# krukah/robopoker

Measured on AMD Instinct MI355X. Metric: mccfr_infoset_updates_per_sec, higher is better.
Workload: dtype f32; 1 GPU; leduc-holdem external-sampling MCCFR, tables resident in HBM (BASELINE configs[1]); regret=floored, weight=linear, sampling=external, batch_per_gpu=8388608, global_batch=8388608, infosets=120, actions=2, update=composed, parallelism=tree-sharded x1

## Files before the change

### robopoker_amd/csrc/mccfr.hip

```cpp
#include "mccfr_kernels.hpp"
#include "mccfr_traverse.hpp"
#include "mccfr_update.hpp"
#include "traverse_static.hpp"
#include "mccfr_nash.hpp"
#include "host_util.hpp"

#include <algorithm>
#include <chrono>
#include <cstdlib>
#include <functional>
#include <string>
#include <type_traits>
#include <vector>

using namespace rp;

namespace {
const char* const CLOCK_NAMES[] = {"traverse", "compact", "update"};
enum { CK_TRAVERSE, CK_COMPACT, CK_UPDATE, CK_COUNT };
}

struct rp_mccfr {
    int device = 0;
    hipStream_t stream = nullptr;
// ... 86 lines not shown
    if (h->d_dec) HIP_TRY(hipFree(h->d_dec));
    h->d_scratch = h->d_dec = nullptr;
    const size_t stride = ((size_t)batch + 255) & ~(size_t)255;
    const uint32_t A = h->tbl.max_actions;
    DevScratch& sc = h->sc;
    sc.stride = stride;
    const size_t node_words = (size_t)sc.maxn * stride, stack_words = (size_t)sc.maxs * stride;
    const size_t total_words = 8 * node_words + 4 * stack_words + (size_t)A * stride;
    HIP_TRY(hipMalloc(&h->d_scratch, total_words * 4));
    uint32_t* base = reinterpret_cast<uint32_t*>(h->d_scratch);
    sc.n_meta = base; base += node_words;
    sc.n_info = base; base += node_words;
    sc.n_frel = reinterpret_cast<float*>(base); base += node_words;
    sc.n_fsmp = reinterpret_cast<float*>(base); base += node_words;
    sc.n_pay = reinterpret_cast<float*>(base); base += node_words;
    sc.n_rel = reinterpret_cast<float*>(base); base += node_words;
    sc.n_smp = reinterpret_cast<float*>(base); base += node_words;
    sc.n_acc = reinterpret_cast<float*>(base); base += node_words;
    sc.s_state = base; base += stack_words;
    sc.s_meta = base; base += stack_words;
    sc.s_frel = reinterpret_cast<float*>(base); base += stack_words;
    sc.s_fsmp = reinterpret_cast<float*>(base); base += stack_words;
    sc.t_v = reinterpret_cast<float*>(base);

    DevDecisions& dc = h->dc;
    dc.stride = stride;
    dc.maxdec = h->maxdec;
    const size_t slot_words = (size_t)dc.maxdec * stride;
    const bool small = chunk_maps_lds_bytes(h) <= 64 * 1024 && h->tbl.n_infos <= CM_PASSES * CH_THREADS && !getenv("RP_MCCFR_SLOTMAP");
    const size_t dec_bytes = (3 * slot_words + 2 * slot_words * A) * 4 + (small ? 0 : (size_t)h->tbl.n_infos * stride) + stride;
    HIP_TRY(hipMalloc(&h->d_dec, dec_bytes));
    uint32_t* d = reinterpret_cast<uint32_t*>(h->d_dec);
    dc.info = d; d += slot_words;
    dc.mask = d; d += slot_words;
    dc.payoff = reinterpret_cast<float*>(d); d += slot_words;
    dc.regret = reinterpret_cast<float*>(d); d += slot_words * A;
    dc.policy = reinterpret_cast<float*>(d); d += slot_words * A;
    dc.ndec = reinterpret_cast<uint8_t*>(d);
    dc.slotmap = small ? nullptr : dc.ndec + stride;
    if (h->d_sorted) HIP_TRY(hipFree(h->d_sorted));
    h->d_sorted = nullptr;
    DevSorted& so = h->so;
    so.n_chunks = (uint32_t)((stride + CH_TREES - 1) / CH_TREES);
    const size_t cap = slot_words;
    const size_t nic = (size_t)h->tbl.n_infos * so.n_chunks;
    const size_t sorted_words = cap * 2 * A + 2 * cap + 2 * nic + h->tbl.n_infos;
    HIP_TRY(hipMalloc(&h->d_sorted, sorted_words * 4));
    uint32_t* sw = reinterpret_cast<uint32_t*>(h->d_sorted);
    so.rw = reinterpret_cast<float*>(sw); sw += cap * 2 * A;
    so.mask = sw; sw += cap;
    so.payoff = reinterpret_cast<float*>(sw); sw += cap;
    so.counts = sw; sw += nic;
    so.offs = sw; sw += nic;
    so.total = sw;
    if (h->d_bmaps) HIP_TRY(hipFree(h->d_bmaps));
    h->d_bmaps = nullptr;
    const size_t nblk_max = (stride + RP_COMPOSE_CHUNK - 1) / RP_COMPOSE_CHUNK;
    const size_t ngrp_max = (nblk_max + RP_FOLD_GROUP - 1) / RP_FOLD_GROUP;
    const size_t bytes = bmap_index((uint32_t)(nblk_max + ngrp_max), 0, 0, h->g.rank_max, 2 * A) * sizeof(Map) + (size_t)h->tbl.n_infos * sizeof(uint32_t);
    HIP_TRY(hipMalloc(&h->d_bmaps, bytes));
    HIP_TRY(hipMemset(h->d_bmaps, 0, bytes));
    HIP_TRY(hipDeviceSynchronize());
    h->capacity = batch;
    return RP_OK;
}

StepParams make_params(const rp_mccfr* h) {
    StepParams p{};
    p.seed = h->seed;
    p.epoch = h->epoch;
    p.tree_base = (uint64_t)h->rank * h->batch;
    p.batch = h->batch;
    p.walker = (uint32_t)(h->epoch % h->tbl.n_players);
    p.R = h->R; p.W = h->W; p.S = h->S;
    p.temperature = h->hp.temperature; p.smoothing = h->hp.smoothing; p.curiosity = h->hp.curiosity;
    p.prune_threshold = h->hp.prune_threshold; p.prune_explore = h->hp.prune_explore;
    p.prune_warmup = h->hp.prune_warmup;
    p.regret_min = h->hp.regret_min;
    if (h->R == RP_REGRET_DISCOUNTED) {
        p.pow15 = rp_pow15((float)h->epoch);
        p.pow05 = rp_pow05((float)h->epoch);
    }
    p.counters = h->d_counters;
    if (h->rng == RP_RNG_REFERENCE) {
        p.ref_info = reinterpret_cast<const rp_sip_mid*>(h->d_ref_mid);
        p.ref_chance = p.ref_info + h->tbl.n_infos;
    }
    return p;
}

template <class F>
void with_bool(bool a, F&& f) {
    if (a) f(std::true_type{});
    else f(std::false_type{});
}
template <class F>
void with_bools(bool a, bool b, F&& f) {
    with_bool(a, [&](auto ta) { with_bool(b, [&](auto tb) { f(ta, tb); }); });
}

template <class F>
void with_skeleton(int static_skel, F&& f) {
    if (static_skel == 1) f(KuhnSkel{});
    else if (static_skel == 2) f(LeducSkel{});
}
template <class F>
void with_static_traversal(int static_skel, uint32_t walker, bool pruned, bool ref, F&& f) {
    with_skeleton(static_skel, [&](auto gt) {
        with_bool(walker == 0, [&](auto w0) {
            with_bools(pruned, ref, [&](auto pr, auto rf) { f(gt, std::integral_constant<int, decltype(w0)::value ? 0 : 1>{}, pr, rf); });
        });
    });
}

template <class G>
bool skel_matches(const rp_game_table* game, const std::vector<uint32_t>& children) {
    constexpr Skeleton S = SkelOf<G>::S;
    if (game->n_players != 2 || game->max_actions != 2) return false;
    std::vector<std::vector<int>> kids(S.n);
    for (int s = 1; s < S.n; ++s) kids[S.parent[s]].push_back(s);
    std::vector<int> node_of_info(game->n_infos, -1);
    std::function<bool(uint32_t, int)> match = [&](uint32_t sid, int s) -> bool {
        const rp_state& st = game->states[sid];
        if (S.kind[s] == SK_TERMINAL) return st.n_children == 0;
        if (S.kind[s] == SK_CHANCE) {
            if (st.turn != RP_TURN_CHANCE || st.n_children == 0 || kids[s].size() != 1) return false;
            for (uint32_t k = 0; k < st.n_children; ++k)
                if (!match(children[st.offset + k], kids[s][0])) return false;
            return true;
        }
        if (st.turn != (uint8_t)(S.kind[s] - SK_P0) || st.n_children != 2 || kids[s].size() != 2 || st.info >= game->n_infos) return false;
        if (node_of_info[st.info] >= 0 && node_of_info[st.info] != s) return false;
        node_of_info[st.info] = s;
        for (int c : kids[s])
            if (S.edge[c] > 1 || !match(children[st.offset + (uint32_t)S.edge[c]], c)) return false;
        return kids[s][0] != kids[s][1] && S.edge[kids[s][0]] != S.edge[kids[s][1]];
    };
    return match(game->train_root, 0);
}

template <class G>
bool build_rows(const rp_game_table* game, const std::vector<uint32_t>& children, const std::function<uint4(uint32_t)>& rec_of,
                std::vector<uint32_t>& rows, uint32_t* base, uint32_t* fan) {
    constexpr Skeleton S = SkelOf<G>::S;
    constexpr RowLayout R = SkelOf<G>::R;
    std::vector<std::vector<int>> kids(S.n);
    for (int s = 1; s < S.n; ++s) kids[S.parent[s]].push_back(s);
    for (int s = 0; s < S.n; ++s) fan[s] = base[s] = 0;
    bool uniform = true;
    std::function<void(uint32_t, int)> fans = [&](uint32_t sid, int s) {
        const rp_state& st = game->states[sid];
        if (S.kind[s] == SK_CHANCE) {
            if (fan[s] == 0) fan[s] = st.n_children;
            else if (fan[s] != st.n_children) uniform = false;
            for (uint32_t k = 0; k < st.n_children; ++k) fans(children[st.offset + k], kids[s][0]);
        } else if (S.kind[s] != SK_TERMINAL) {
            for (int c : kids[s]) fans(children[st.offset + (uint32_t)S.edge[c]], c);
        }
    };
    fans(game->train_root, 0);
    if (!uniform) return false;
    uint64_t total = 0;
    for (int c = 0; c < S.n; ++c) {
        if (S.kind[c] != SK_CHANCE) continue;
        uint64_t count = 1;
        for (int a = 0; a <= c; ++a)
            if (S.kind[a] == SK_CHANCE && c <= S.end[a]) count *= fan[a];
        base[c] = (uint32_t)(total / 4);
        total += (count * (uint64_t)R.stride[c] + 31) & ~(uint64_t)31;
        if (total > (1ull << 28)) return false;
    }
    rows.assign(total, 0u);
    std::function<void(uint32_t, int, uint64_t)> fill = [&](uint32_t sid, int s, uint64_t idx) {
        const rp_state& st = game->states[sid];
        if (const int c = R.group[s]; c >= 0) {
            uint32_t* row = &rows[(size_t)base[c] * 4 + idx * (uint64_t)R.stride[c]];
            const uint4 r = rec_of(sid);
            if (S.kind[s] == SK_CHANCE) {
                row[R.word[s]] = r.w;
                row[R.word2[s]] = r.y;
            } else if (S.kind[s] == SK_TERMINAL) {
                row[R.word[s]] = r.y;
                row[R.word2[s]] = r.z;
            } else {
                row[R.word[s]] = r.y;
            }
        }
        if (S.kind[s] == SK_CHANCE) {
            for (uint32_t k = 0; k < st.n_children; ++k) fill(children[st.offset + k], kids[s][0], idx * fan[s] + k);
        } else if (S.kind[s] != SK_TERMINAL) {
            for (int c : kids[s]) fill(children[st.offset + (uint32_t)S.edge[c]], c, idx);
        }
    };
    fill(game->train_root, 0, 0);
    return true;
}

size_t traverse_lds_bytes(const rp_mccfr* h) {
    const size_t shared = std::max<size_t>(2 * (size_t)h->maxint, 4 * (size_t)h->sc.maxs);
    return ((size_t)2 * h->sc.maxn + shared + (h->tbl.max_actions <= 4 ? 0 : h->tbl.max_actions)) * 64 * 4;
}
bool traverse_fits_lds(const rp_mccfr* h) {
    return h->sc.maxn <= 62 && h->maxint <= 32 && h->tbl.max_depth <= 10 && h->tbl.n_infos <= 8191 && h->tbl.max_actions <= 16 &&
           traverse_lds_bytes(h) <= 64 * 1024;
}

void launch_prepare_ref(rp_mccfr* h, const StepParams& p) {
    if (h->rng == RP_RNG_REFERENCE && h->ref_mid_epoch != p.epoch) {
        const uint32_t n = h->tbl.n_infos + h->n_chance_infos;
        rp_sip_mid* mid = reinterpret_cast<rp_sip_mid*>(h->d_ref_mid);
        hipLaunchKernelGGL(k_prepare_ref, dim3((n + 63) / 64), dim3(64), 0, h->stream, reinterpret_cast<const rp_hash_stream*>(h->d_info_streams),
                           h->tbl.n_infos, reinterpret_cast<const rp_hash_stream*>(h->d_chance_streams), h->n_chance_infos, p.epoch, mid,
                           mid + h->tbl.n_infos);
        h->ref_mid_epoch = p.epoch;
    }
}
void launch_prepare(rp_mccfr* h, const StepParams& p) {
    launch_prepare_ref(h, p);
    if (h->itab_version == h->tables_version) return;
    hipLaunchKernelGGL(k_prepare_infos, dim3((h->tbl.n_infos + 63) / 64), dim3(64), 0, h->stream, h->g, h->t, p, h->itab);
    h->itab_version = h->tables_version;
}

int launch_traverse(rp_mccfr* h, const StepParams& p) {
    if (h->dc.slotmap) HIP_TRY(hipMemsetAsync(h->dc.slotmap, 0, (size_t)h->tbl.n_infos * h->dc.stride, h->stream));
    h->clk.begin(h->stream, CK_TRAVERSE);
    if (h->static_skel) {
        launch_prepare(h, p);
        const dim3 grid((h->batch + 255) / 256), block(256);
        with_static_traversal(h->static_skel, p.walker, p.S != RP_SAMPLING_EXTERNAL, p.ref_info != nullptr, [&](auto gt, auto wk, auto pr, auto rf) {
            hipLaunchKernelGGL((k_traverse_static<decltype(gt), decltype(wk)::value, decltype(pr)::value, decltype(rf)::value>), grid, block, 0,
                               h->stream, h->g, h->itab, h->dc, p);
        });
    } else if (h->use_lds_traverse) {
        launch_prepare(h, p);
        const size_t lds = traverse_lds_bytes(h);
        const dim3 grid((h->batch + 63) / 64), block(64);
        with_bool(h->tbl.max_actions <= 4, [&](auto tv) {
            hipLaunchKernelGGL((k_traverse_lds<decltype(tv)::value>), grid, block, lds, h->stream, h->g, h->itab, h->dc, p, h->sc.maxn, h->sc.maxs,
                               h->maxint);
        });
    } else {
        launch_prepare_ref(h, p);
        const uint32_t threads = 256, blocks = (h->batch + threads - 1) / threads;
        hipLaunchKernelGGL(k_traverse, dim3(blocks), dim3(threads), 0, h->stream, h->g, h->t, h->sc, h->dc, p);
    }
    h->clk.end(h->stream, CK_TRAVERSE);
    HIP_TRY(hipGetLastError());
    return RP_OK;
}

int launch_sort(rp_mccfr* h, const StepParams& p) {
    const uint32_t nchunks = (h->batch + CH_TREES - 1) / CH_TREES;
    h->so.n_chunks = nchunks;
    h->clk.begin(h->stream, CK_COMPACT);
    if (!h->dc.slotmap) {
        const size_t NI = h->tbl.n_infos;
        hipLaunchKernelGGL(k_count_small, dim3(nchunks), dim3(CH_THREADS), NI * SM_WORDS * 4, h->stream, h->g, h->dc, h->so, p);
        hipLaunchKernelGGL(k_scan, dim3(h->tbl.n_infos), dim3(CH_THREADS), 0, h->stream, h->g, h->so, p);
        hipLaunchKernelGGL(k_compact_small, dim3(nchunks), dim3(CH_THREADS), NI * SM_WORDS * 4 + 2 * NI * 4 + NI * SM_WORDS * 2,
                           h->stream, h->g, h->dc, h->so, p);
    } else {
        hipLaunchKernelGGL(k_count, dim3(nchunks, h->tbl.n_infos), dim3(SLOT_THREADS), 0, h->stream, h->g, h->dc, h->so, p);
        hipLaunchKernelGGL(k_scan, dim3(h->tbl.n_infos), dim3(CH_THREADS), 0, h->stream, h->g, h->so, p);
        hipLaunchKernelGGL(k_compact, dim3(nchunks, h->tbl.n_infos), dim3(SLOT_THREADS), 0, h->stream, h->g, h->dc, h->so, p);
    }
    h->clk.end(h->stream, CK_COMPACT);
    HIP_TRY(hipGetLastError());
    return RP_OK;
}

int launch_chain(rp_mccfr* h, const StepParams& p) {
    const size_t lds = chain_lds_bytes();
    const bool sgn = h->R == RP_REGRET_DISCOUNTED || h->R == RP_REGRET_ASYMMETRIC;
    const bool prn = h->S != RP_SAMPLING_EXTERNAL;
    const dim3 grid(h->tbl.n_infos), block(128);
    h->clk.begin(h->stream, CK_UPDATE);
    with_bools(sgn, prn, [&](auto sg, auto pr) {
        hipLaunchKernelGGL((k_chain<decltype(sg)::value, decltype(pr)::value>), grid, block, lds, h->stream, h->g, h->t, h->so, p);
    });
    h->clk.end(h->stream, CK_UPDATE);
    HIP_TRY(hipGetLastError());
    return RP_OK;
}

uint32_t chunks_of(size_t trees) { return (uint32_t)((trees + RP_COMPOSE_CHUNK - 1) / RP_COMPOSE_CHUNK); }
size_t chunk_maps_lds_bytes(const rp_mccfr* h) {
    const size_t NI = h->tbl.n_infos;
    return NI * SM_WORDS * 4 + 2 * NI * 4 + (size_t)CH_TREES * h->maxdec * 4 + NI * SM_WORDS * 2 +
           2 * (size_t)CH_TREES * h->maxdec * 2;
}

size_t traverse_maps_lds_bytes(const rp_mccfr* h) {
    const size_t NI = h->tbl.n_infos;
    const size_t masks = h->S != RP_SAMPLING_EXTERNAL ? (size_t)h->maxdec * 256 * 4 : 0;
    return (NI * 8 + 2 * NI) * 4 + NI * 8 * 2 + (NI + (NI & 1)) * 2 + 2 * NI * 4 + (size_t)3 * (h->maxdec * 256 + h->cell_pad) * 4 + masks;
}
static_assert(CH_THREADS <= 256u, "k_traverse_maps_static packs (infoset, rank of the infoset) into the 16 bits of an `order` entry");
bool traverse_maps_fused(const rp_mccfr* h) {
    return h->static_skel && !h->dc.slotmap && h->tbl.n_infos <= CH_THREADS && h->g.rank_max <= 64u &&
           traverse_maps_lds_bytes(h) <= 64 * 1024 && h->fuse_maps;
}

constexpr uint32_t FOLD_SPLIT_GROUPS = 128;
bool fold_split(const rp_mccfr* h, uint32_t batch) {
    const uint32_t ngrp = (chunks_of(batch) + RP_FOLD_GROUP - 1) / RP_FOLD_GROUP;
    return ngrp >= h->fold_split_groups;
}

int launch_summarize(rp_mccfr* h, const StepParams& p, void* blob_dev, bool fused = false, bool apply = false) {
    unsigned char* blob = reinterpret_cast<unsigned char*>(blob_dev);
    Cell* cells = reinterpret_cast<Cell*>(blob);
    InfoSum* sums = reinterpret_cast<InfoSum*>(blob + (size_t)h->tbl.n_infos * h->tbl.max_actions * sizeof(Cell));
    const uint32_t A = h->tbl.max_actions;
    const uint32_t nblk_max = chunks_of(h->dc.stride), nblk = chunks_of(h->batch);
    Map* bmaps = reinterpret_cast<Map*>(h->d_bmaps);
    const bool pruned = h->S != RP_SAMPLING_EXTERNAL;
    if (fused) {
        h->clk.begin(h->stream, CK_TRAVERSE);
        launch_prepare(h, p);
        const size_t lds = traverse_maps_lds_bytes(h);
        with_static_traversal(h->static_skel, p.walker, pruned, p.ref_info != nullptr, [&](auto gt, auto wk, auto pr, auto rf) {
            hipLaunchKernelGGL((k_traverse_maps_static<decltype(gt), decltype(wk)::value, decltype(pr)::value, decltype(rf)::value>), dim3(nblk),
                               dim3(256), lds, h->stream, h->g, h->itab, p, bmaps, h->maxdec, h->cell_pad);
        });
        h->clk.end(h->stream, CK_TRAVERSE);
    }
    h->clk.begin(h->stream, CK_UPDATE);
    if (fused) {
    } else if (!h->dc.slotmap) {
        const size_t lds = chunk_maps_lds_bytes(h);
        with_bools(pruned, h->tbl.n_infos <= CH_THREADS, [&](auto pr, auto one) {
            hipLaunchKernelGGL((k_chunk_maps<decltype(pr)::value, decltype(one)::value ? 1u : CM_PASSES>), dim3(nblk), dim3(CH_THREADS), lds,
                               h->stream, h->g, h->dc, p, bmaps);
        });
    } else {
        with_bool(pruned, [&](auto pr) {
            hipLaunchKernelGGL((k_block_maps<decltype(pr)::value>), dim3(nblk, h->tbl.n_infos), dim3(128), 0, h->stream, h->g, h->so, p, bmaps);
        });
    }
    {
        const uint32_t W2 = 2 * A, nr = h->g.rank_count[p.walker];
        const uint32_t ngrp_max = (nblk_max + RP_FOLD_GROUP - 1) / RP_FOLD_GROUP, ngrp = (nblk + RP_FOLD_GROUP - 1) / RP_FOLD_GROUP;
        FoldScratch fs;
        fs.gmaps = bmaps + bmap_index(nblk_max, 0, 0, h->g.rank_max, W2);
        fs.done = reinterpret_cast<uint32_t*>(bmaps + bmap_index(nblk_max + ngrp_max, 0, 0, h->g.rank_max, W2));
        const dim3 grid(std::max(ngrp, 1u), cb2_tiles(nr, W2)), fold_grid(std::max(nr, 1u));
        const bool split = fold_split(h, h->batch);
        if (split) hipLaunchKernelGGL((k_combine2<false, false>), grid, dim3(CB2_THREADS), 0, h->stream, h->g, h->t, h->itab, p, bmaps, nr, fs, cells, sums);
        if (apply) {
            if (split) hipLaunchKernelGGL((k_fold_groups<true>), fold_grid, dim3(CB2_THREADS), 0, h->stream, h->g, h->t, h->itab, p, fs.gmaps, nr, cells, sums);
            else hipLaunchKernelGGL((k_combine2<true>), grid, dim3(CB2_THREADS), 0, h->stream, h->g, h->t, h->itab, p, bmaps, nr, fs, cells, sums);
            h->tables_version += 1;
            if (h->itab_version + 1 == h->tables_version) h->itab_version = h->tables_version;
        } else {
            if (split) hipLaunchKernelGGL((k_fold_groups<false>), fold_grid, dim3(CB2_THREADS), 0, h->stream, h->g, h->t, h->itab, p, fs.gmaps, nr, cells, sums);
            else hipLaunchKernelGGL((k_combine2<false>), grid, dim3(CB2_THREADS), 0, h->stream, h->g, h->t, h->itab, p, bmaps, nr, fs, cells, sums);
        }
    }
    h->clk.end(h->stream, CK_UPDATE);
    HIP_TRY(hipGetLastError());
    return RP_OK;
}

int launch_batch_summary(rp_mccfr* h, const StepParams& p, void* blob_dev, bool apply = false) {
    if (traverse_maps_fused(h)) return launch_summarize(h, p, blob_dev, true, apply);
    int rc = launch_traverse(h, p);
    if (rc) return rc;
    if (h->dc.slotmap && (rc = launch_sort(h, p))) return rc;
    return launch_summarize(h, p, blob_dev, false, apply);
}

int enqueue_step(rp_mccfr* h) {
    const StepParams p = make_params(h);
    int rc;
    if (h->mode == RP_UPDATE_ORDERED) {
        if ((rc = launch_traverse(h, p))) return rc;
        if ((rc = launch_sort(h, p))) return rc;
        if ((rc = launch_chain(h, p))) return rc;
        h->tables_version += 1;
    } else {
        if ((rc = launch_batch_summary(h, p, h->d_summary, true))) return rc;
    }
    h->epoch += 1;
    return RP_OK;
}

int read_counters(rp_mccfr* h, unsigned long long c[3]) {
    std::vector<unsigned long long> all((size_t)METRIC_STRIPES * METRIC_STRIDE);
    HIP_TRY(hipMemcpyAsync(all.data(), h->d_counters, all.size() * 8, hipMemcpyDeviceToHost, h->stream));
    HIP_TRY(hipStreamSynchronize(h->stream));
    c[0] = c[1] = c[2] = 0;
    for (uint32_t s = 0; s < METRIC_STRIPES; ++s) {
        c[0] += all[(size_t)s * METRIC_STRIDE];
        c[1] += all[(size_t)s * METRIC_STRIDE + 1];
        c[2] |= all[(size_t)s * METRIC_STRIDE + 2];
    }
    return RP_OK;
}

int check_device_errors(rp_mccfr* h) {
    unsigned long long c[3];
    int rc = read_counters(h, c);
    if (rc) return rc;
    if (c[2]) return rp::fail(RP_ERR_CAPACITY, "mccfr kernel capacity exceeded (flags %llu): nodes/stack/decisions", c[2]);
    return RP_OK;
}

int composed_supported(const rp_mccfr* h) {
    if (h->R == RP_REGRET_DISCOUNTED || h->R == RP_REGRET_ASYMMETRIC)
        return rp::fail(RP_ERR_UNSUPPORTED,
                        "composed update needs a sign-independent discount (Summed/Linear/Floored regret)");
    return RP_OK;
}

int fetch_tables(rp_mccfr* h, std::vector<float>& regret, std::vector<float>& weight, std::vector<float>& payoff,
                 std::vector<uint32_t>& visits) {
    const size_t cells = (size_t)h->tbl.n_infos * h->tbl.max_actions;
    regret.resize(cells); weight.resize(cells); payoff.resize(cells); visits.resize(cells);
    HIP_TRY(hipMemcpyAsync(regret.data(), h->t.regret, cells * 4, hipMemcpyDeviceToHost, h->stream));
    HIP_TRY(hipMemcpyAsync(weight.data(), h->t.weight, cells * 4, hipMemcpyDeviceToHost, h->stream));
    HIP_TRY(hipMemcpyAsync(payoff.data(), h->t.payoff, cells * 4, hipMemcpyDeviceToHost, h->stream));
    HIP_TRY(hipMemcpyAsync(visits.data(), h->t.visits, cells * 4, hipMemcpyDeviceToHost, h->stream));
    HIP_TRY(hipStreamSynchronize(h->stream));
    return RP_OK;
}

}

extern "C" {

int rp_mccfr_create(const rp_game_table* game, rp_regret_kind r, rp_weight_kind w, rp_sampling_kind s,
                    uint32_t batch_size, const rp_hyper* hp, uint64_t seed, int device, rp_mccfr** out) {
    if (!game || !out) return rp::fail(RP_ERR_INVALID, "rp_mccfr_create: NULL argument");
    int rc = rp_game_table_check(game);
    if (rc) return rc;
    if ((int)r < 0 || (int)r > 4 || (int)w < 0 || (int)w > 3 || (int)s < 0 || (int)s > 2)
        return rp::fail(RP_ERR_INVALID, "rp_mccfr_create: unknown schedule / sampling kind");
    if (batch_size == 0) return rp::fail(RP_ERR_INVALID, "rp_mccfr_create: batch_size must be > 0");
    if (rp_device_count() <= 0)
        return rp::fail(RP_ERR_NO_DEVICE, "rp_mccfr_create: no HIP device visible; the MI355X path has no CPU fallback");
    if (game->max_tree_nodes == 0 || game->max_tree_nodes >= 255)
        return rp::fail(RP_ERR_CAPACITY, "rp_mccfr_create: sampled trees of up to %u nodes exceed the per-lane limit (254)",
                        game->max_tree_nodes);
    rp_mccfr* h = new rp_mccfr();
    h->device = device;
    h->tbl = *game;
    h->states.assign(game->states, game->states + game->n_states);
    h->children.assign(game->children, game->children + game->n_children);
    h->payoffs.assign(game->payoffs, game->payoffs + (size_t)game->n_terminals * game->n_players);
    h->info_actions.assign(game->info_actions, game->info_actions + game->n_infos);
    h->info_player.assign(game->info_player, game->info_player + game->n_infos);
    const size_t cells = (size_t)game->n_infos * game->max_actions;
    h->default_regret.assign(cells, 0.0f);
    if (game->default_regret) h->default_regret.assign(game->default_regret, game->default_regret + cells);
    h->tbl.states = h->states.data();
    h->tbl.children = h->children.data();
    h->tbl.payoffs = h->payoffs.data();
    h->tbl.info_actions = h->info_actions.data();
    h->tbl.info_player = h->info_player.data();
    h->tbl.default_regret = h->default_regret.data();
    h->R = r; h->W = w; h->S = s;
    if (hp) h->hp = *hp; else rp_hyper_default(&h->hp);
    h->seed = seed;
    h->batch = batch_size;

#define CREATE_TRY(expr)                                                                             \
    do {                                                                                             \
        hipError_t _e = (expr);                                                                      \
        if (_e != hipSuccess) {                                                                      \
            int _rc = rp::fail(RP_ERR_HIP, "%s failed: %s", #expr, hipGetErrorString(_e));           \
            rp_mccfr_destroy(h);                                                                     \
            return _rc;                                                                              \
        }                                                                                            \
    } while (0)

    CREATE_TRY(hipSetDevice(device));
    CREATE_TRY(hipStreamCreateWithFlags(&h->stream, hipStreamNonBlocking));
    h->own_stream = true;
    std::vector<uint4> packed(game->n_states);
    for (uint32_t i = 0; i < game->n_states; ++i) {
        const rp_state& st = game->states[i];
        packed[i] = make_uint4((uint32_t)st.turn | ((uint32_t)st.n_children << 8), st.turn == RP_TURN_CHANCE ? (uint32_t)st.chance_info : st.info, st.offset, 0u);
    }
    CREATE_TRY(hipMalloc(&h->d_states, packed.size() * sizeof(uint4)));
    CREATE_TRY(hipMemcpy(h->d_states, packed.data(), packed.size() * sizeof(uint4), hipMemcpyHostToDevice));
    CREATE_TRY(hipMalloc(&h->d_children, h->children.size() * 4));
    CREATE_TRY(hipMemcpy(h->d_children, h->children.data(), h->children.size() * 4, hipMemcpyHostToDevice));
    const std::function<uint4(uint32_t)> rec_of = [&](uint32_t sid) {
        uint4 r = packed[sid];
        r.w = sid;
        if (game->states[sid].n_children == 0 && game->n_players == 2) {
            r.y = rp_f2u(h->payoffs[(size_t)game->states[sid].offset * 2 + 0]);
            r.z = rp_f2u(h->payoffs[(size_t)game->states[sid].offset * 2 + 1]);
        }
        return r;
    };
    std::vector<uint4> kids(h->children.size());
    for (size_t c = 0; c < h->children.size(); ++c) kids[c] = rec_of(h->children[c]);
    CREATE_TRY(hipMalloc(&h->d_kids, std::max<size_t>(kids.size(), 1) * sizeof(uint4)));
    CREATE_TRY(hipMemcpy(h->d_kids, kids.data(), kids.size() * sizeof(uint4), hipMemcpyHostToDevice));
    CREATE_TRY(hipMalloc(&h->d_payoffs, h->payoffs.size() * 4));
    CREATE_TRY(hipMemcpy(h->d_payoffs, h->payoffs.data(), h->payoffs.size() * 4, hipMemcpyHostToDevice));
    CREATE_TRY(hipMalloc(&h->d_info_actions, game->n_infos));
    CREATE_TRY(hipMemcpy(h->d_info_actions, h->info_actions.data(), game->n_infos, hipMemcpyHostToDevice));
    CREATE_TRY(hipMalloc(&h->d_info_player, game->n_infos));
    CREATE_TRY(hipMemcpy(h->d_info_player, h->info_player.data(), game->n_infos, hipMemcpyHostToDevice));
    h->g.states = reinterpret_cast<const uint4*>(h->d_states);
    h->g.children = reinterpret_cast<const uint32_t*>(h->d_children);
    h->g.kids = reinterpret_cast<const uint4*>(h->d_kids);
    h->g.root_rec = packed[game->train_root];
    h->g.root_rec.w = game->train_root;
    h->g.payoffs = reinterpret_cast<const float*>(h->d_payoffs);
    h->g.info_actions = reinterpret_cast<const uint8_t*>(h->d_info_actions);
    h->g.info_player = reinterpret_cast<const uint8_t*>(h->d_info_player);
    {
        std::vector<uint32_t> rank(game->n_infos), count(8, 0u);
        const auto owned = [&](uint32_t i) { return h->info_player[i] < game->n_players; };
        for (uint32_t i = 0; i < game->n_infos; ++i) rank[i] = owned(i) ? count[h->info_player[i]]++ : 0u;
        uint32_t rank_max = 1;
        for (uint32_t w = 0; w < 8; ++w) {
            h->g.rank_count[w] = count[w];
            rank_max = std::max(rank_max, count[w]);
        }
        h->g.rank_max = rank_max;
        std::vector<uint32_t> tab((size_t)game->n_infos + (size_t)game->n_players * rank_max, 0u);
        for (uint32_t i = 0; i < game->n_infos; ++i) {
            tab[i] = rank[i];
            if (owned(i)) tab[(size_t)game->n_infos + (size_t)h->info_player[i] * rank_max + rank[i]] = i;
        }
        CREATE_TRY(hipMalloc(&h->d_info_rank, tab.size() * 4));
        CREATE_TRY(hipMemcpy(h->d_info_rank, tab.data(), tab.size() * 4, hipMemcpyHostToDevice));
        h->g.info_rank = reinterpret_cast<const uint32_t*>(h->d_info_rank);
        h->g.rank_info = h->g.info_rank + game->n_infos;
    }
    h->g.n_players = game->n_players;
    h->g.n_infos = game->n_infos;
    h->g.A = game->max_actions;
    h->g.root = game->train_root;
    CREATE_TRY(hipMalloc(&h->t.regret, cells * 4));
    CREATE_TRY(hipMalloc(&h->t.weight, cells * 4));
    CREATE_TRY(hipMalloc(&h->t.payoff, cells * 4));
    CREATE_TRY(hipMalloc(&h->t.visits, cells * 4));
    CREATE_TRY(hipMemcpy(h->t.regret, h->default_regret.data(), cells * 4, hipMemcpyHostToDevice));
    CREATE_TRY(hipMemset(h->t.weight, 0, cells * 4));
    CREATE_TRY(hipMemset(h->t.payoff, 0, cells * 4));
    CREATE_TRY(hipMemset(h->t.visits, 0, cells * 4));
    CREATE_TRY(hipMalloc(&h->d_counters, (size_t)METRIC_STRIPES * METRIC_STRIDE * sizeof(unsigned long long)));
    CREATE_TRY(hipMemset(h->d_counters, 0, (size_t)METRIC_STRIPES * METRIC_STRIDE * sizeof(unsigned long long)));
    CREATE_TRY(hipMalloc(&h->d_summary, summary_bytes_of(h)));
    CREATE_TRY(hipMalloc(&h->d_itab, (5 * cells + 2 * (size_t)game->n_infos + 4 + 8 * (size_t)game->n_infos + 8) * 4));
    {
        float* f = reinterpret_cast<float*>(h->d_itab);
        h->itab.sigma = f;
        h->itab.q = f + cells;
        h->itab.cum = f + 2 * cells;
        h->itab.total = f + 3 * cells;
        h->itab.keep = reinterpret_cast<uint32_t*>(f + 3 * cells + game->n_infos);
        const size_t used = 3 * cells + 2 * (size_t)game->n_infos;
        h->itab.sq = reinterpret_cast<float2*>(f + ((used + 3) & ~(size_t)3));
        const size_t used2 = ((used + 3) & ~(size_t)3) + 2 * cells;
        h->itab.row2 = game->max_actions == 2 ? f + ((used2 + 7) & ~(size_t)7) : nullptr;
    }
    uint32_t maxstack = 1;
    sampled_tree_bounds(h, &h->maxdec, &maxstack, &h->maxint);
    h->sc.maxn = game->max_tree_nodes;
    h->sc.maxs = maxstack;
    if (h->maxdec > 254) {
        rp_mccfr_destroy(h);
        return rp::fail(RP_ERR_CAPACITY, "rp_mccfr_create: more than 254 walker infosets per tree");
    }
    if (chain_lds_bytes() > 64 * 1024) {
        rp_mccfr_destroy(h);
        return rp::fail(RP_ERR_CAPACITY, "rp_mccfr_create: chain tiles need %zu B of LDS", chain_lds_bytes());
    }
    h->use_lds_traverse = traverse_fits_lds(h) && getenv("RP_MCCFR_HBM_SCRATCH") == nullptr;
    h->fuse_maps = getenv("RP_TRAV_UNFUSED") == nullptr;
    const char* fold_env = getenv("RP_FOLD_SPLIT");
    h->fold_split_groups = !fold_env ? FOLD_SPLIT_GROUPS : (atoi(fold_env) ? 1u : UINT32_MAX);
    if (h->use_lds_traverse && getenv("RP_TRAV_GENERIC") == nullptr) {
        for (int k = 1; k <= 2 && !h->static_skel; ++k)
            with_skeleton(k, [&](auto gt) {
                if (skel_matches<decltype(gt)>(game, h->children)) h->static_skel = k;
            });
    }
    h->g.rows = nullptr;
    if (h->static_skel && getenv("RP_TRAV_NO_FLAT") == nullptr) {
        std::vector<uint32_t> rows;
        bool ok = false;
        with_skeleton(h->static_skel, [&](auto gt) { ok = build_rows<decltype(gt)>(game, h->children, rec_of, rows, h->g.row_base, h->g.row_fan); });
        if (ok) {
            CREATE_TRY(hipMalloc(&h->d_rows, rows.size() * 4));
            CREATE_TRY(hipMemcpy(h->d_rows, rows.data(), rows.size() * 4, hipMemcpyHostToDevice));
            h->g.rows = reinterpret_cast<const uint4*>(h->d_rows);
            h->rows_bytes = rows.size() * 4;
        }
    }
    rc = alloc_batch_buffers(h, batch_size);
    if (rc) {
        rp_mccfr_destroy(h);
        return rc;
    }
#undef CREATE_TRY
    (void)hipDeviceSynchronize();
    *out = h;
    return RP_OK;
}
// ... 726 lines not shown
```

### robopoker_amd/csrc/mccfr_update.hpp

```cpp
#ifndef RP_MCCFR_UPDATE_HPP
#define RP_MCCFR_UPDATE_HPP

#include "mccfr_kernels.hpp"
#include "mccfr_traverse.hpp"

namespace rp {

#define CH_THREADS 256u
#define SLOT_THREADS (CH_TREES / 4u)

__device__ __forceinline__ uint32_t chunk_slots(const DevDecisions& dc, uint32_t info, uint32_t t0, uint32_t batch) {
    uint32_t slots = 0;
    if (t0 + 4 <= batch) {
        slots = *reinterpret_cast<const uint32_t*>(&dc.slotmap[(size_t)info * dc.stride + t0]);
    } else {
        for (uint32_t k = 0; k < 4; ++k)
            if (t0 + k < batch) slots |= (uint32_t)dc.slotmap[(size_t)info * dc.stride + t0 + k] << (8 * k);
    }
    return slots;
}
__device__ __forceinline__ uint32_t nonzero_bytes(uint32_t v) {
    return ((v & 0xffu) != 0) + ((v & 0xff00u) != 0) + ((v & 0xff0000u) != 0) + ((v & 0xff000000u) != 0);
}
__device__ __forceinline__ uint32_t block_exscan(uint32_t v, uint32_t* wave_tot, uint32_t* total) {
// ... 426 lines not shown
}

template <bool PRUNED>
__global__ __launch_bounds__(128) void k_block_maps(DevGame g, DevSorted so, StepParams p, Map* bmaps) {
    __shared__ __attribute__((aligned(16))) float tile[TILE_FLOATS + 2 * RP_MAX_ACTIONS * TILE_PAD];
    __shared__ uint32_t mtile[TILE_FLOATS / 2];
    __shared__ __attribute__((aligned(16))) float ptile[TILE_FLOATS / 2];
    const uint32_t info = blockIdx.y, blk = blockIdx.x;
    if (g.info_player[info] != p.walker) return;
    const uint32_t A = g.A, nact = g.info_actions[info], W2 = 2 * A;
    const uint32_t T = compose_block(A);
    const uint32_t n = so.counts[(size_t)info * so.n_chunks + blk];
    const uint32_t TP = T + TILE_PAD;
    const uint32_t wave = threadIdx.x >> 6, lane = threadIdx.x & 63u;
    const size_t base = seg_base(so, info) + so.offs[(size_t)info * so.n_chunks + blk];
    const bool isreg = lane < A;
    const uint32_t a = lane % A;
    const bool chain = lane < W2 && a < nact;
    const float tf = (float)p.epoch;
    const ChainParams cp = chain_params(p, isreg, tf);
    const float fl = cp.fl, d = cp.d;
    Map mp{1.0f, 0.0f, rp_u2f(0xff800000u), 0u};
    float psum = 0.0f;
    for (uint32_t t0 = 0; t0 < n; t0 += T) {
        const uint32_t m = min(T, n - t0);
        if (wave == 0) {
            const size_t e0 = (base + t0) * W2;
            const uint32_t nfl = m * W2;
            float lr[TILE_FLOATS / 64];
#pragma unroll
            for (uint32_t q = 0; q < TILE_FLOATS / 64; ++q) {
                const uint32_t k = lane + 64 * q;
                lr[q] = k < nfl ? so.rw[e0 + k] : 0.0f;
            }
#pragma unroll
            for (uint32_t q = 0; q < TILE_FLOATS / 64; ++q) {
                const uint32_t k = lane + 64 * q;
                if (k < nfl) tile[(k % W2) * TP + k / W2] = lr[q];
            }
            if (PRUNED)
                for (uint32_t k = lane; k < m; k += 64) mtile[k] = so.mask[base + t0 + k];
        } else {
            for (uint32_t k = lane; k < m; k += 64) ptile[k] = so.payoff[base + t0 + k];
        }
        __syncthreads();
        if (wave == 0 && chain) {
            const float* row = tile + lane * TP;
            for (uint32_t i = 0; i < m; ++i) {
                const float delta = row[i];
                const bool skip = PRUNED && isreg && !((mtile[i] >> a) & 1u);
                const float na = mp.n ? mp.a * d : d;
                const float nb = mp.n ? mp.b * d + delta : delta;
                const float nm = mp.n ? rp_maxf(mp.m * d + delta, fl) : fl;
                mp.a = skip ? mp.a : na;
                mp.b = skip ? mp.b : nb;
                mp.m = skip ? mp.m : nm;
                mp.n += skip ? 0u : 1u;
            }
        }
        if (wave == 1 && lane == 0)
            for (uint32_t i = 0; i < m; ++i) psum += ptile[i];
        __syncthreads();
    }
    const size_t out = bmap_index(blk, g.info_rank[info], 0u, g.rank_max, W2);
    if (wave == 0 && lane < W2) bmaps[out + lane] = Map{mp.a, mp.b, mp.m, chain ? mp.n : 0u};
    if (wave == 1 && lane == 0) bmaps[out + W2] = map_sum_slot(psum, n);
}

template <bool PRUNED, uint32_t PASSES>
__global__ __launch_bounds__(CH_THREADS) void k_chunk_maps(DevGame g, DevDecisions dc, StepParams p, Map* bmaps) {
    extern __shared__ __attribute__((aligned(16))) uint32_t cm_lds[];
    __shared__ uint32_t wave_tot[CH_THREADS / 64];
    const uint32_t NI = g.n_infos, A = g.A, W2 = 2 * A, chunk = blockIdx.x, tid = threadIdx.x, MD = dc.maxdec;
    uint32_t* bits = cm_lds;
    uint32_t* lcount = bits + NI * SM_WORDS;
    uint32_t* lbase = lcount + NI;
    float* vals = reinterpret_cast<float*>(lbase + NI);
    uint16_t* pre = reinterpret_cast<uint16_t*>(vals + MD * CH_TREES);
    uint16_t* posl = pre + NI * SM_WORDS;
    uint16_t* lmask = posl + MD * CH_TREES;
    chunk_bitmap(dc, NI, chunk, p.batch, bits);
    for (uint32_t info = tid; info < NI; info += CH_THREADS) lcount[info] = list_prefix(bits, pre, info);
    __syncthreads();
    lds_exscan(lcount, lbase, NI, wave_tot);
    const uint32_t lt = tid, tree = chunk * CH_TREES + lt;
    const uint32_t nd = tree < p.batch ? dc.ndec[tree] : 0u;
    for (uint32_t slot = 0; slot < nd; ++slot) {
        const uint32_t info = dc.info[slot * dc.stride + tree];
        const uint32_t pos = lbase[info] + list_rank(bits, pre, info, lt);
        posl[slot * CH_TREES + lt] = (uint16_t)pos;
        if (PRUNED) lmask[pos] = (uint16_t)dc.mask[slot * dc.stride + tree];
    }
    const float tf = (float)p.epoch;
    uint32_t my_nact[PASSES], my_n[PASSES], my_base[PASSES];
#pragma unroll
    for (uint32_t q = 0; q < PASSES; ++q) {
        const uint32_t info = tid + q * CH_THREADS;
        const bool mine = info < NI && g.info_player[info < NI ? info : 0u] == p.walker;
        my_nact[q] = mine ? g.info_actions[info] : 0u;
        my_n[q] = mine ? lcount[info] : 0u;
        my_base[q] = mine ? lbase[info] : 0u;
    }
    for (uint32_t c = 0; c <= W2; ++c) {
        const bool isreg = c < A, ispay = c == W2;
        const uint32_t a = c % A;
        __syncthreads();
        for (uint32_t slot = 0; slot < nd; ++slot) {
            float v;
            if (ispay) v = dc.payoff[slot * dc.stride + tree];
            else if (isreg) v = dc.regret[(slot * A + a) * dc.stride + tree];
            else v = weight_delta(p.W, dc.policy[(slot * A + a) * dc.stride + tree], tf);
            vals[posl[slot * CH_TREES + lt]] = v;
        }
        __syncthreads();
#pragma unroll
        for (uint32_t q = 0; q < PASSES; ++q) {
            const uint32_t info = tid + q * CH_THREADS;
            if (!my_nact[q]) continue;
            const uint32_t n = my_n[q], base = my_base[q];
            const size_t out = bmap_index(chunk, g.info_rank[info], c, g.rank_max, W2);
            if (ispay) {
                float sum = 0.0f;
                for (uint32_t e = 0; e < n; ++e) sum += vals[base + e];
                bmaps[out] = map_sum_slot(sum, n);
                continue;
            }
            const bool chain = a < my_nact[q];
            const ChainParams cp = chain_params(p, isreg, tf);
            Map mp = map_identity();
            if (chain)
                for (uint32_t e = 0; e < n; ++e)
                    map_touch_unless(mp, PRUNED && isreg && !((lmask[base + e] >> a) & 1u), cp.d, vals[base + e], cp.fl);
            bmaps[out] = mp;
        }
    }
}

#if defined(__HIP_DEVICE_COMPILE__) && !defined(__gfx950__) && !defined(__gfx942__)
#error "k_combine2's cross-workgroup hand-over relies on gfx942/gfx950 store counting and sc1 semantics: use an acq_rel arrival counter on other targets"
#endif
__device__ __forceinline__ void st_agent(uint32_t* q, uint32_t v) { __hip_atomic_store(q, v, __ATOMIC_RELAXED, __HIP_MEMORY_SCOPE_AGENT); }
__device__ __forceinline__ void st_map(Map* m, const Map& v) {
    uint32_t* w = reinterpret_cast<uint32_t*>(m);
    st_agent(w, rp_f2u(v.a));
    st_agent(w + 1, rp_f2u(v.b));
    st_agent(w + 2, rp_f2u(v.m));
    st_agent(w + 3, v.n);
}
#ifndef CB2_DEPTH
#define CB2_DEPTH 8u
#endif
#ifndef CB2_DEPTH2
#define CB2_DEPTH2 8u
#endif
#define CB2_THREADS 256u
static_assert(2u * RP_MAX_ACTIONS + 1u <= CB2_THREADS, "a tile of k_combine2 holds at least one whole infoset");
__host__ __device__ inline uint32_t cb2_tile_infos(uint32_t W2) { return CB2_THREADS / (W2 + 1u); }
__host__ __device__ inline uint32_t cb2_tiles(uint32_t nr, uint32_t W2) { return nr ? (nr + cb2_tile_infos(W2) - 1u) / cb2_tile_infos(W2) : 1u; }
struct FoldScratch {
    Map* gmaps;
    uint32_t* done;
};
template <uint32_t D, class Load>
__device__ __forceinline__ Map fold_slots(Map m, uint32_t n, bool sum, Load load) {
    uint4 va[D], vb[D];
    auto issue = [&](uint4* v, uint32_t k0) __attribute__((always_inline)) {
#pragma unroll
        for (uint32_t q = 0; q < D; ++q) v[q] = load(min(k0 + q, n - 1u));
    };
    auto fold = [&](const uint4* v, uint32_t k0) __attribute__((always_inline)) {
#pragma unroll
        for (uint32_t q = 0; q < D; ++q) {
            const Map s{rp_u2f(v[q].x), rp_u2f(v[q].y), rp_u2f(v[q].z), v[q].w};
            const Map c = map_compose_select(m, s);
            const bool on = k0 + q < n;
            m.a = on ? c.a : m.a;
            m.b = on ? (sum ? m.b + s.b : c.b) : m.b;
            m.m = on ? c.m : m.m;
            m.n = on ? m.n + s.n : m.n;
        }
    };
    uint32_t k0 = 0;
    issue(va, 0u);
    for (; k0 + 2u * D < n; k0 += 2u * D) {
        issue(vb, k0 + D);
        __builtin_amdgcn_sched_barrier(0);
        fold(va, k0);
        __builtin_amdgcn_sched_barrier(0);
        issue(va, k0 + 2u * D);
        __builtin_amdgcn_sched_barrier(0);
        fold(vb, k0 + D);
        __builtin_amdgcn_sched_barrier(0);
    }
    if (k0 + D < n) {
        issue(vb, k0 + D);
        __builtin_amdgcn_sched_barrier(0);
        fold(va, k0);
        fold(vb, k0 + D);
    } else {
        fold(va, k0);
    }
    return m;
}
__device__ __forceinline__ void blob_idle_entries(const DevGame& g, const StepParams& p, Cell* cells, InfoSum* sums) {
    const uint32_t A = g.A, W2 = 2 * A, SL = W2 + 1u;
    const Map ident = map_identity();
    for (uint32_t e = threadIdx.x; e < g.n_infos * SL; e += CB2_THREADS) {
        const uint32_t info = e / SL, slot = e - info * SL;
        if (g.info_player[info] == p.walker) continue;
        if (slot == W2) {
            sums[info] = InfoSum{0u, 0.0f};
        } else {
            Cell& cl = cells[(size_t)info * A + slot % A];
            if (slot < A) cell_set_regret(cl, ident);
            else cell_set_weight(cl, ident);
        }
    }
}
template <bool APPLY>
__device__ __forceinline__ void fold_finish(const DevGame& g, const DevTables& t, const DevInfoTab& it, const StepParams& p, bool active, uint32_t li,
                                            uint32_t slot, uint32_t info, const Map& tot, Cell* cells, InfoSum* sums, float* sh_ps, uint32_t* sh_len) {
    const uint32_t A = g.A, W2 = 2 * A;
    const bool sum = slot == W2;
    if (!APPLY) {
        if (active) {
            if (sum) {
                sums[info] = InfoSum{tot.n, tot.b};
            } else {
                Cell& cl = cells[(size_t)info * A + slot % A];
                if (slot < A) cell_set_regret(cl, tot);
                else cell_set_weight(cl, tot);
            }
        }
        return;
    }
    if (active && sum) {
        sh_ps[li] = tot.b;
        sh_len[li] = tot.n;
    }
    __syncthreads();
    if (active && !sum && slot % A < g.info_actions[info]) {
        const uint32_t cell = info * A + slot % A;
        if (slot < A) {
            t.regret[cell] = map_apply(tot, t.regret[cell]);
            float ev = t.payoff[cell];
            uint32_t visits = t.visits[cell];
            fold_payoff(ev, visits, sh_ps[li], sh_len[li]);
            t.payoff[cell] = ev;
            t.visits[cell] = visits;
        } else {
            t.weight[cell] = map_apply(tot, t.weight[cell]);
        }
    }
    __syncthreads();
    if (active && slot == 0) prepare_one(g, t, p, it, info);
}
template <bool APPLY, bool TAIL = true>
__global__ __launch_bounds__(CB2_THREADS) void k_combine2(DevGame g, DevTables t, DevInfoTab it, StepParams p, const Map* bmaps, uint32_t nr,
                                                          FoldScratch fs, Cell* cells, InfoSum* sums) {
    static_assert(TAIL || !APPLY, "stage 1 alone applies nothing");
    __shared__ uint32_t role;
    __shared__ float sh_ps[CB2_THREADS / 3u];
    __shared__ uint32_t sh_len[CB2_THREADS / 3u];
    const uint32_t grp = blockIdx.x, tile = blockIdx.y, tid = threadIdx.x;
    const uint32_t A = g.A, W2 = 2 * A, SL = W2 + 1u;
    if (TAIL && !APPLY && grp == 0 && tile == 0) blob_idle_entries(g, p, cells, sums);
    const uint32_t nb = (p.batch + RP_COMPOSE_CHUNK - 1) / RP_COMPOSE_CHUNK;
    const uint32_t ngrp = (nb + RP_FOLD_GROUP - 1) / RP_FOLD_GROUP;
    if (grp >= ngrp) return;
    const uint32_t ntiles = cb2_tiles(nr, W2);
    const uint32_t r_lo = (uint32_t)((uint64_t)tile * nr / ntiles), r_hi = (uint32_t)((uint64_t)(tile + 1u) * nr / ntiles);
    const uint32_t li = tid / SL, slot = tid - li * SL, rank = r_lo + li;
    const bool active = rank < r_hi, sum = slot == W2;
    const size_t row = (size_t)g.rank_max * SL;
    if (active) {
        const uint32_t b_lo = grp * RP_FOLD_GROUP, n = min(nb, b_lo + RP_FOLD_GROUP) - b_lo;
        const uint4* src = reinterpret_cast<const uint4*>(bmaps) + bmap_index(b_lo, rank, slot, g.rank_max, W2);
        const Map m = fold_slots<CB2_DEPTH>(map_identity(), n, sum, [&](uint32_t k) { return src[(size_t)k * row]; });
        if (TAIL) st_map(&fs.gmaps[bmap_index(grp, rank, slot, g.rank_max, W2)], m);
        else fs.gmaps[bmap_index(grp, rank, slot, g.rank_max, W2)] = m;
    }
    if (!TAIL) return;
    asm volatile("s_waitcnt vmcnt(0)" ::: "memory");
    __syncthreads();
    if (tid == 0) role = atomicAdd(&fs.done[tile], 1u) == ngrp - 1u ? 1u : 0u;
    __syncthreads();
    if (!role) return;
    if (tid == 0) fs.done[tile] = 0;
    Map tot = map_identity();
    uint32_t info = 0;
    if (active) {
        const uint64_t* gm = reinterpret_cast<const uint64_t*>(fs.gmaps + bmap_index(0u, rank, slot, g.rank_max, W2));
        tot = fold_slots<CB2_DEPTH2>(tot, ngrp, sum, [&](uint32_t k) {
            const uint64_t* w = gm + (size_t)k * row * 2u;
            const uint64_t lo = __hip_atomic_load(w, __ATOMIC_RELAXED, __HIP_MEMORY_SCOPE_AGENT);
            const uint64_t hi = __hip_atomic_load(w + 1, __ATOMIC_RELAXED, __HIP_MEMORY_SCOPE_AGENT);
            return make_uint4((uint32_t)lo, (uint32_t)(lo >> 32), (uint32_t)hi, (uint32_t)(hi >> 32));
        });
        info = g.rank_info[(size_t)p.walker * g.rank_max + rank];
    }
    fold_finish<APPLY>(g, t, it, p, active, li, slot, info, tot, cells, sums, sh_ps, sh_len);
}

#define FG_LOADS 10u
#define FG_SLOTS (FG_LOADS * CB2_THREADS)
#define FG_DEPTH 8u
static_assert(2u * RP_MAX_ACTIONS + 1u <= FG_SLOTS, "a slab of k_fold_groups holds at least one group");
__host__ __device__ inline uint32_t fg_slab_groups(uint32_t W2) { return FG_SLOTS / (W2 + 1u); }
template <bool APPLY>
__global__ __launch_bounds__(CB2_THREADS) void k_fold_groups(DevGame g, DevTables t, DevInfoTab it, StepParams p, const Map* gmaps, uint32_t nr,
                                                             Cell* cells, InfoSum* sums) {
    typedef uint32_t __attribute__((ext_vector_type(4))) Word4;
    __shared__ __attribute__((aligned(16))) Word4 slab[FG_SLOTS];
    __shared__ float sh_ps[1];
    __shared__ uint32_t sh_len[1];
    const uint32_t rank = blockIdx.x, tid = threadIdx.x;
    const uint32_t A = g.A, W2 = 2 * A, SL = W2 + 1u;
    if (!APPLY && rank == 0) blob_idle_entries(g, p, cells, sums);
    if (rank >= nr) return;
    const uint32_t nb = (p.batch + RP_COMPOSE_CHUNK - 1) / RP_COMPOSE_CHUNK;
    const uint32_t ngrp = (nb + RP_FOLD_GROUP - 1) / RP_FOLD_GROUP, per = fg_slab_groups(W2);
    const size_t row = (size_t)g.rank_max * SL;
    const Word4* src = reinterpret_cast<const Word4*>(gmaps) + bmap_index(0u, rank, 0u, g.rank_max, W2);
    const bool active = tid < SL;
    Map tot = map_identity();
    for (uint32_t g0 = 0; g0 < ngrp; g0 += per) {
        const uint32_t n = min(per, ngrp - g0), nel = n * SL;
        Word4 v[FG_LOADS];
#pragma unroll
        for (uint32_t q = 0; q < FG_LOADS; ++q) {
            const uint32_t e = min(tid + q * CB2_THREADS, nel - 1u), k = e / SL;
            v[q] = src[(size_t)(g0 + k) * row + (e - k * SL)];
        }
        if (g0) __syncthreads();
#pragma unroll
        for (uint32_t q = 0; q < FG_LOADS; ++q) {
            const uint32_t e = tid + q * CB2_THREADS;
            if (e < nel) slab[e] = v[q];
        }
        __syncthreads();
        if (active) tot = fold_slots<FG_DEPTH>(tot, n, tid == W2, [&](uint32_t k) {
            const Word4 w = slab[k * SL + tid];
            return make_uint4(w.x, w.y, w.z, w.w);
        });
    }
    const uint32_t info = g.rank_info[(size_t)p.walker * g.rank_max + rank];
    fold_finish<APPLY>(g, t, it, p, active, 0u, tid, info, tot, cells, sums, sh_ps, sh_len);
}

__global__ void k_fold(DevGame g, DevTables t, const unsigned char* blob, size_t blob_stride, uint32_t world) {
    const uint32_t cell = blockIdx.x * blockDim.x + threadIdx.x;
    const uint32_t ncell = g.n_infos * g.A;
    if (cell >= ncell) return;
    const uint32_t info = cell / g.A, a = cell % g.A;
    if (a >= g.info_actions[info]) return;
    float r = t.regret[cell], w = t.weight[cell], ev = t.payoff[cell];
    uint32_t visits = t.visits[cell];
    for (uint32_t rk = 0; rk < world; ++rk) {
        const unsigned char* b = blob + (size_t)rk * blob_stride;
        const Cell c = reinterpret_cast<const Cell*>(b)[cell];
        const InfoSum s = reinterpret_cast<const InfoSum*>(b + (size_t)ncell * sizeof(Cell))[info];
        if (c.rn) r = map_eval(cell_regret(c), r);
        if (c.wn) w = map_eval(cell_weight(c), w);
        fold_payoff(ev, visits, s.psum, s.count);
    }
    t.regret[cell] = r;
    t.weight[cell] = w;
    t.payoff[cell] = ev;
    t.visits[cell] = visits;
}

__global__ void k_accumulate(DevGame g, unsigned char* acc, const unsigned char* step, uint32_t first) {
    const uint32_t cell = blockIdx.x * blockDim.x + threadIdx.x;
    const uint32_t ncell = g.n_infos * g.A;
    if (cell >= ncell) return;
    const Cell s = reinterpret_cast<const Cell*>(step)[cell];
    Cell* ac = reinterpret_cast<Cell*>(acc) + cell;
    if (first) {
        *ac = s;
    } else {
        const Cell a = *ac;
        const Map r = map_compose(cell_regret(a), cell_regret(s));
        const Map w = map_compose(cell_weight(a), cell_weight(s));
        *ac = Cell{r.a, r.b, r.m, w.a, w.b, w.m, r.n, w.n};
    }
    if (cell % g.A == 0) {
        const uint32_t info = cell / g.A;
        const InfoSum si = reinterpret_cast<const InfoSum*>(step + (size_t)ncell * sizeof(Cell))[info];
        InfoSum* ai = reinterpret_cast<InfoSum*>(acc + (size_t)ncell * sizeof(Cell)) + info;
        if (first) *ai = si;
        else *ai = InfoSum{ai->count + si.count, ai->psum + si.psum};
    }
}

}

#endif
```

Measured before the change: 86.00 billion infoset-updates/s.

## Add unit-slope fast path to group fold with compacted operand lists

Within k_fold_groups, each slab checks block-wide whether every map operand has unit slope (a==1). If so, it compacts the non-empty operands per slot into LDS with ballot/mbcnt and folds them with a simpler add/max recurrence that is software-pipelined across two register buffers. The payoff lane's sum moves to a separate wavefront. It also lowers the threshold for taking the split fold path, which adds extra ballots, LDS traffic and syncs and costs more when the general path is needed.

```diff
diff --git a/robopoker_amd/csrc/mccfr.hip b/robopoker_amd/csrc/mccfr.hip
--- a/robopoker_amd/csrc/mccfr.hip
+++ b/robopoker_amd/csrc/mccfr.hip
@@ -412,7 +412,7 @@
            traverse_maps_lds_bytes(h) <= 64 * 1024 && h->fuse_maps;
 }
 
-constexpr uint32_t FOLD_SPLIT_GROUPS = 128;
+constexpr uint32_t FOLD_SPLIT_GROUPS = 64;
 bool fold_split(const rp_mccfr* h, uint32_t batch) {
     const uint32_t ngrp = (chunks_of(batch) + RP_FOLD_GROUP - 1) / RP_FOLD_GROUP;
     return ngrp >= h->fold_split_groups;
diff --git a/robopoker_amd/csrc/mccfr_update.hpp b/robopoker_amd/csrc/mccfr_update.hpp
--- a/robopoker_amd/csrc/mccfr_update.hpp
+++ b/robopoker_amd/csrc/mccfr_update.hpp
@@ -752,19 +752,84 @@
     fold_finish<APPLY>(g, t, it, p, active, li, slot, info, tot, cells, sums, sh_ps, sh_len);
 }
 
+typedef float __attribute__((ext_vector_type(2))) FgOp;
+__device__ __forceinline__ bool unit_operand(uint32_t a, uint32_t b, uint32_t m) {
+    return a == 0x3f800000u && (b & 0x7f800000u) != 0x7f800000u && (m & 0x7fffffffu) <= 0x7f800000u;
+}
+template <uint32_t D>
+__device__ __forceinline__ void fold_unit_ops(Map& tot, const FgOp* op, uint32_t cnt, uint32_t nsum) {
+    float B = tot.b, M = tot.m;
+    uint32_t k = 0;
+    if (tot.n == 0 && cnt) {
+        B = op[0].x;
+        M = op[0].y;
+        k = 1;
+    }
+    FgOp va[D], vb[D];
+    auto issue = [&](FgOp* v, uint32_t k0) __attribute__((always_inline)) {
+#pragma unroll
+        for (uint32_t q = 0; q < D; ++q) v[q] = op[k0 + q];
+    };
+    auto fold = [&](const FgOp* v) __attribute__((always_inline)) {
+#pragma unroll
+        for (uint32_t q = 0; q < D; ++q) {
+            B = B + v[q].x;
+            M = rp_maxf(M + v[q].x, v[q].y);
+        }
+    };
+    if (k + D <= cnt) {
+        issue(va, k);
+        for (; k + 3u * D <= cnt; k += 2u * D) {
+            issue(vb, k + D);
+            __builtin_amdgcn_sched_barrier(0);
+            fold(va);
+            __builtin_amdgcn_sched_barrier(0);
+            issue(va, k + 2u * D);
+            __builtin_amdgcn_sched_barrier(0);
+            fold(vb);
+            __builtin_amdgcn_sched_barrier(0);
+        }
+        if (k + 2u * D <= cnt) {
+            issue(vb, k + D);
+            __builtin_amdgcn_sched_barrier(0);
+            fold(va);
+            fold(vb);
+            k += 2u * D;
+        } else {
+            fold(va);
+            k += D;
+        }
+    }
+    for (; k < cnt; ++k) {
+        const FgOp v = op[k];
+        B = B + v.x;
+        M = rp_maxf(M + v.x, v.y);
+    }
+    tot.b = B;
+    tot.m = M;
+    tot.n += nsum;
+}
 #define FG_LOADS 10u
 #define FG_SLOTS (FG_LOADS * CB2_THREADS)
 #define FG_DEPTH 8u
+#define FG_WAVES (CB2_THREADS / 64u)
+#define FG_PAY_LANE (CB2_THREADS - 64u)
 static_assert(2u * RP_MAX_ACTIONS + 1u <= FG_SLOTS, "a slab of k_fold_groups holds at least one group");
+static_assert(2u * RP_MAX_ACTIONS <= FG_PAY_LANE, "the cell lanes of k_fold_groups end before its payoff lane's wavefront");
 __host__ __device__ inline uint32_t fg_slab_groups(uint32_t W2) { return FG_SLOTS / (W2 + 1u); }
 template <bool APPLY>
 __global__ __launch_bounds__(CB2_THREADS) void k_fold_groups(DevGame g, DevTables t, DevInfoTab it, StepParams p, const Map* gmaps, uint32_t nr,
                                                              Cell* cells, InfoSum* sums) {
     typedef uint32_t __attribute__((ext_vector_type(4))) Word4;
     __shared__ __attribute__((aligned(16))) Word4 slab[FG_SLOTS];
+    __shared__ __attribute__((aligned(8))) FgOp ops[FG_SLOTS];
+    __shared__ uint32_t op_cnt[2u * RP_MAX_ACTIONS], op_n[2u * RP_MAX_ACTIONS];
+    __shared__ uint32_t sh_general[FG_WAVES];
+    __shared__ float pay_b;
+    __shared__ uint32_t pay_n;
     __shared__ float sh_ps[1];
     __shared__ uint32_t sh_len[1];
-    const uint32_t rank = blockIdx.x, tid = threadIdx.x;
+    const uint32_t rank = blockIdx.x, tid = threadIdx.x, wave = tid >> 6, lane = tid & 63u;
     const uint32_t A = g.A, W2 = 2 * A, SL = W2 + 1u;
     if (!APPLY && rank == 0) blob_idle_entries(g, p, cells, sums);
     if (rank >= nr) return;
@@ -777,22 +842,77 @@
     for (uint32_t g0 = 0; g0 < ngrp; g0 += per) {
         const uint32_t n = min(per, ngrp - g0), nel = n * SL;
         Word4 v[FG_LOADS];
+        uint32_t vslot[FG_LOADS];
 #pragma unroll
         for (uint32_t q = 0; q < FG_LOADS; ++q) {
             const uint32_t e = min(tid + q * CB2_THREADS, nel - 1u), k = e / SL;
-            v[q] = src[(size_t)(g0 + k) * row + (e - k * SL)];
+            vslot[q] = e - k * SL;
+            v[q] = src[(size_t)(g0 + k) * row + vslot[q]];
         }
         if (g0) __syncthreads();
+        bool general = tid < W2 && tot.n != 0u && !unit_operand(rp_f2u(tot.a), rp_f2u(tot.b), rp_f2u(tot.m));
 #pragma unroll
         for (uint32_t q = 0; q < FG_LOADS; ++q) {
             const uint32_t e = tid + q * CB2_THREADS;
             if (e < nel) slab[e] = v[q];
-        }
+            general |= vslot[q] != W2 && v[q].w != 0u && !unit_operand(v[q].x, v[q].y, v[q].z);
+        }
+        const bool wave_general = __ballot(general) != 0ull;
+        if (lane == 0) sh_general[wave] = wave_general ? 1u : 0u;
         __syncthreads();
-        if (active) tot = fold_slots<FG_DEPTH>(tot, n, tid == W2, [&](uint32_t k) {
-            const Word4 w = slab[k * SL + tid];
-            return make_uint4(w.x, w.y, w.z, w.w);
-        });
+        uint32_t any_general = 0;
+#pragma unroll
+        for (uint32_t w = 0; w < FG_WAVES; ++w) any_general |= sh_general[w];
+        if (__builtin_amdgcn_readfirstlane(any_general)) {
+            if (active) tot = fold_slots<FG_DEPTH>(tot, n, tid == W2, [&](uint32_t k) {
+                const Word4 w = slab[k * SL + tid];
+                return make_uint4(w.x, w.y, w.z, w.w);
+            });
+            continue;
+        }
+        for (uint32_t s = wave; s < W2; s += FG_WAVES) {
+            uint32_t base = 0, nsum = 0;
+            for (uint32_t k0 = 0; k0 < n; k0 += 64u) {
+                const uint32_t k = k0 + lane;
+                const Word4 w = slab[min(k, n - 1u) * SL + s];
+                const bool on = k < n && w.w != 0u;
+                const uint64_t mask = __ballot(on);
+                if (on) {
+                    const uint32_t at = base + __builtin_amdgcn_mbcnt_hi((uint32_t)(mask >> 32), __builtin_amdgcn_mbcnt_lo((uint32_t)mask, 0u));
+                    ops[s * n + at] = FgOp{rp_u2f(w.y), rp_u2f(w.z)};
+                    nsum += w.w;
+                }
+                base += (uint32_t)__popcll(mask);
+            }
+            for (int d = 32; d > 0; d >>= 1) nsum += __shfl_xor(nsum, d, 64);
+            if (lane == 0) {
+                op_cnt[s] = base;
+                op_n[s] = nsum;
+            }
+        }
+        if (tid == W2) {
+            pay_b = tot.b;
+            pay_n = tot.n;
+        }
+        __syncthreads();
+        if (tid < W2) fold_unit_ops<FG_DEPTH>(tot, ops + tid * n, op_cnt[tid], op_n[tid]);
+        if (tid == FG_PAY_LANE) {
+            float b = pay_b;
+            uint32_t cn = pay_n;
+#pragma unroll 8
+            for (uint32_t k = 0; k < n; ++k) {
+                const Word4 w = slab[k * SL + W2];
+                b += rp_u2f(w.y);
+                cn += w.w;
+            }
+            pay_b = b;
+            pay_n = cn;
+        }
+        __syncthreads();
+        if (tid == W2) {
+            tot.b = pay_b;
+            tot.n = pay_n;
+        }
     }
     const uint32_t info = g.rank_info[(size_t)p.walker * g.rank_max + rank];
     fold_finish<APPLY>(g, t, it, p, active, 0u, tid, info, tot, cells, sums, sh_ps, sh_len);
```

Measured after the change: 91.50 billion infoset-updates/s, median of 6. 6.4% higher.
